# TianyiFranklinWang/MIRROR

Hardware: AMD Instinct MI355X
Metric: SSL samples/sec (slide+RNA pairs) (higher is better)
Workload: dtype bf16; 1 GPU; BASELINE c2: B=16/GPU x [4096 patch tokens x 1024-d] + [2048 genes], D=512, RNA depth 6 / 8 heads, train mode, local-batch InfoNCE; precision_policy=bf16, per_gpu_batch=16, global_batch=16, parallelism=dp1, grad_bucket_dtype=f32, step_launch=hip_graph

## Files before the change

### include/mirror_hip.h

```cpp
#ifndef MIRROR_HIP_H
#define MIRROR_HIP_H
#include <stdint.h>

#ifdef __cplusplus
extern "C" {
#endif

#define MH_OK 0
#define MH_EINVAL (-1)
#define MH_EUNSUP (-2)
#define MH_EHIP (-3)

#define MH_F32 0
#define MH_BF16 1

#define MH_ACT_NONE 0
#define MH_ACT_RELU 1
#define MH_ACT_GELU 2

typedef void* mh_stream;

const char* mh_last_error(void);
int mh_version(void);
int mh_exp_build(void);
// ... 122 lines not shown
                   int dt_v, int dt_o, mh_stream s);
int mh_resconv_wgrad(const void* v, int64_t ldv, int64_t v_bs, const void* dout, int64_t ldo, int64_t o_bs,
                     float* dw, int B, int n_p, int heads, int dh, int taps, int dt_v, int dt_o, mh_stream s);
int64_t mh_resconv_bwd_workspace_bytes(int B, int n_p, int heads, int dh, int taps);
int mh_resconv_bwd(const void* dout, int64_t ldo, int64_t o_bs, const void* v, int64_t ldv, int64_t v_bs, const float* w, void* dv,
                   int64_t lddv, int64_t dv_bs, float* dw, float* workspace, int64_t ws_floats, int B, int n_p, int heads, int dh,
                   int taps, int dt_v, int dt_o, mh_stream s);
int mh_pinv_absmax(const float* x, uint64_t* stats64, int BH, int m, mh_stream s);
int mh_pinv_z0(const float* x, const uint64_t* stats64, float* z0, int BH, int m, mh_stream s);
int mh_pinv_z0_bwd(const float* x, const float* z0, const float* dz0, const uint64_t* stats64, float* dx,
                   float* scratch1, int scratch_zeroed, int BH, int m, mh_stream s);
int mh_pinv_s2_bwd(const float* p, const float* dz0, const uint64_t* stats64, float* dx, float* scratch1, int scratch_zeroed, int BH,
                   int m, const float* mlm, int heads, mh_stream s);
int mh_pinv_chain_prep(const float* x, const uint64_t* stats64, float* z0, void* xp, void* z0p, int BH, int m, mh_stream s);
int mh_pinv_chain_pack(const float* dz, void* up, int BH, int m, mh_stream s);
int mh_pinv_chain_fwd(const void* XP, void* saved, void* zfT, int BH, int m, int iters, const float* z0f, const uint64_t* stats64,
                      int z0_rowmajor, mh_stream s);
int mh_nys_sim2(const void* lm, float* a2, void* xp, float* z0f, uint64_t* stats64, int B, int m, int D, int heads, float scale,
                int64_t lm_ld, const float* mlm, mh_stream s);
int mh_nys_dz_dav(const float* dw2, const float* av, const void* zfT, void* up, void* dav, float* delta3, int BH, int m, int dh,
                  mh_stream s);
int mh_pinv_chain_bwd(const void* XP, const void* saved, const void* dzf, void* work, float* dX, float* dz0, int BH, int m,
                      int iters, mh_stream s);
int64_t mh_pinv_chain_workspace_bytes(int BH, int m, int iters, int which);
int mh_nys_attn1_fwd(const void* qkv, const void* lm, const void* w2, void* out, float* lse1, const float* mrow, const float* mlm,
                     int B, int h, int n_p, int m, int dh, float scale, int accumulate, int64_t lm_ld, void* o1, mh_stream s);
int mh_nys_attn1_fwd_q8(const void* qkv, const void* lm, const void* w2, void* out, float* lse1, int B, int h, int n_p, int m, int dh,
                        float scale, int accumulate, void* q8, unsigned* ring, const float* tick, float margin, float* q8_scale, void* o1,
                        mh_stream s);
int64_t mh_nys_attn3_ws_floats(int B, int h, int n_p);
int64_t mh_nys_attn3_workspace_bytes(int B, int h, int n_p);
int mh_nys_attn3_fwd(const void* qkv, const void* lm, float* av, float* lse3, float* workspace, int64_t ws_floats,
                     const float* mrow, const float* mlm, int B, int h, int n_p, int m, int dh, float scale, int64_t lm_ld,
                     const float* rc_w, void* rc_out, mh_stream s);
int mh_nys_attn1_bwd(const void* qkv, const void* lm, const void* w2, const void* dout, const float* lse1, const void* o1, float* delta1,
                     void* dqkv, float* dw2, float* dlm, const float* mrow, const float* mlm, int B, int h, int n_p, int m, int dh,
                     float scale, int64_t lm_ld, mh_stream s);
int mh_nys_attn3_bwd(const void* qkv, const void* lm, const float* av, const void* dav, const float* lse3, float* delta3,
                     void* dqkv, float* dlm, const float* mrow, const float* mlm, int B, int h, int n_p, int m, int dh,
                     float scale, int64_t lm_ld, mh_stream s);
int mh_nys_cls_attn(const void* qkv, const void* lm, const void* z, const float* lse3, float* row, const float* mrow, const float* mlm,
                    int B, int h, int n_p, int m, int dh, int cls_row, float scale, int64_t lm_ld, int z_colmajor, int dt,
                    mh_stream s);
int mh_lm_merge(const float* a, const float* b, void* out, int64_t rows, int cols, int64_t out_ld, int zero_cols, mh_stream s);
int mh_eye_minus(const float* P, float* T, float d, int BH, int m, mh_stream s);

// ... 240 lines not shown
```

### mirror_amd/_lib.py

```python
from __future__ import annotations

import ctypes as C
import os

_HERE = os.path.dirname(os.path.abspath(__file__))
LIB_PATH = os.environ.get("MIRROR_HIP_LIB") or os.path.join(_HERE, "lib", "libmirror_hip.so")

MH_F32, MH_BF16 = 0, 1
ACT_NONE, ACT_RELU, ACT_GELU = 0, 1, 2


class GemmEpi(C.Structure):
    _fields_ = [
        ("kind", C.c_int32), ("resid", C.c_void_p),
        ("p", C.c_float), ("seed", C.c_uint64), ("offset", C.c_uint64), ("dev_base", C.c_void_p),
        ("mask", C.c_void_p), ("token", C.c_void_p), ("pos", C.c_void_p),
        ("rows_per_batch", C.c_int32), ("first", C.c_int32),
        ("tgt", C.c_void_p), ("tgt_bs", C.c_int64), ("sq", C.c_void_p),
    ]


class SkinnyWgradItem(C.Structure):
    _fields_ = [("dy", C.c_void_p), ("lddy", C.c_int64), ("x", C.c_void_p), ("ldx", C.c_int64), ("dw", C.c_void_p), ("lddw", C.c_int64),
                ("db", C.c_void_p), ("M", C.c_int32), ("N", C.c_int32), ("K", C.c_int32), ("dt_dy", C.c_int32), ("dt_x", C.c_int32)]
# ... 82 lines not shown
    "mh_layernorm_bwd": [P, P, P, P, P, P, P, P, I, I, I, L, L, I, I, I, I, P, L],
    "mh_layernorm_bwd_fan": [P, P, P, P, P, P, P, P, I, I, I, L, L, I, I, P, L, P, F, P],
    "mh_layernorm_bwd_drop": [P, P, P, P, P, P, P, P, I, I, I, L, L, I, I, P, L, P, F, P, P, F, U64, U64, P, P, I],
    "mh_layernorm_bwd_lm": [P, P, P, P, P, P, P, P, I, I, I, L, L, I, I, I, I, P, L, P, I, I, P, I, I, P, P, P],
    "mh_layernorm_fwd_lm": [P, P, P, P, P, P, P, P, I, I, I, L, I, I, F, P, P],
    "mh_softmax_fwd": [P, P, L, I, L, L, I, I],
    "mh_softmax_bwd": [P, P, P, L, I, L, L, L, I, I, I],
    "mh_landmark_fwd": [P, P, I, I, I, I, I],
    "mh_landmark_bwd": [P, P, I, I, I, I, I],
    "mh_resconv_fwd": [P, L, L, P, P, L, L, I, I, I, I, I, I, I, I, I],
    "mh_resconv_wgrad": [P, L, L, P, L, L, P, I, I, I, I, I, I, I],
    "mh_resconv_bwd": [P, L, L, P, L, L, P, P, L, L, P, P, L, I, I, I, I, I, I, I],
    "mh_pinv_absmax": [P, P, I, I],
    "mh_pinv_z0": [P, P, P, I, I],
    "mh_pinv_z0_bwd": [P, P, P, P, P, P, I, I, I],
    "mh_pinv_s2_bwd": [P, P, P, P, P, I, I, I, P, I],
    "mh_eye_minus": [P, P, F, I, I],
    "mh_pinv_chain_prep": [P, P, P, P, P, I, I],
    "mh_pinv_chain_pack": [P, P, I, I],
    "mh_pinv_chain_fwd": [P, P, P, I, I, I, P, P, I],
    "mh_nys_sim2": [P, P, P, P, P, I, I, I, I, F, L, P],
    "mh_nys_dz_dav": [P, P, P, P, P, P, I, I, I],
    "mh_pinv_chain_bwd": [P, P, P, P, P, P, I, I, I],
    "mh_nys_attn1_fwd": [P, P, P, P, P, P, P, I, I, I, I, I, F, I, L, P],
    "mh_nys_attn1_fwd_q8": [P, P, P, P, P, I, I, I, I, I, F, I, P, P, P, F, P, P],
    "mh_nys_attn3_fwd": [P, P, P, P, P, L, P, P, I, I, I, I, I, F, L, P, P],
    "mh_nys_attn1_bwd": [P, P, P, P, P, P, P, P, P, P, P, P, I, I, I, I, I, F, L],
    "mh_nys_attn3_bwd": [P, P, P, P, P, P, P, P, P, P, I, I, I, I, I, F, L],
    "mh_nys_cls_attn": [P, P, P, P, P, P, P, I, I, I, I, I, I, F, L, I, I],
    "mh_seq_finish": [P, P, I, I, I, I, I],
    "mh_seq_finish_bwd": [P, P, I, I, I, I, I],
    "mh_ppeg_merge": [P, P, P, P, P, P, P, P, I],
    "mh_ppeg_fwd": [P, P, P, P, I, I, I, I, I, I],
    "mh_ppeg_wgrad": [P, P, P, P, I, I, I, I, I],
    "mh_ppeg_grad_scatter": [P, P, P, P, P, P, P, P, I],
    "mh_rank_mask": [P, P, I, I, I],
    "mh_mask_apply_fwd": [P, P, P, P, P, I, I, I, I, I, I, I],
    "mh_mask_apply_bwd": [P, P, P, P, P, I, I, I, I, I, I, I, P],
    "mh_headattn_fwd": [P, P, P, I, I, I, I],
    "mh_headattn_bwd": [P, P, P, P, I, I, I, I],
    "mh_add": [P, P, P, L, I, I, I],
    "mh_lm_merge": [P, P, P, L, I, L, I],
    "mh_cast": [P, P, L, I, I],
    "mh_gelu_fwd": [P, P, L, I, I],
    "mh_gelu_bwd": [P, P, P, L, I, I, I],
    "mh_relu_bwd": [P, P, P, L, I, L, L, L, I, I, I],
# ... 161 lines not shown
```

### mirror_amd/csrc/nystrom_sim2.hip

```cpp
#include <cstdlib>
#include "gemm_kernel.h"

namespace {

#ifndef SIM2_EXP
#define SIM2_EXP 0
#endif
constexpr int SM = 256;
constexpr int SDH = 64;
constexpr long SMAT = (long)SM * SM;

template <int CTRL>
__device__ __forceinline__ float dpp_f(float v) {
    return __builtin_bit_cast(float, __builtin_amdgcn_update_dpp(0, __builtin_bit_cast(int, v), CTRL, 0xf, 0xf, true));
}
__device__ __forceinline__ float swz16_f(float v) {
    return __builtin_bit_cast(float, __builtin_amdgcn_ds_swizzle(__builtin_bit_cast(int, v), 0x401F));
}
__device__ __forceinline__ float half_max(float v) {
    v = fmaxf(v, dpp_f<0xB1>(v));
    v = fmaxf(v, dpp_f<0x4E>(v));
    v = fmaxf(v, dpp_f<0x141>(v));
    v = fmaxf(v, dpp_f<0x140>(v));
    return fmaxf(v, swz16_f(v));
// ... 153 lines not shown
#pragma unroll
            for (int e = 0; e < 16; e++) c[e] = __builtin_amdgcn_exp2f(c[e] * sl2 - mxi) * ivi;
#pragma unroll
            for (int t = 0; t < 2; t++) {
                float* dst = z0b + ((long)(cb * 16 + 2 * (2 * wave + rb) + t) * 64 + lane) * 8;
                *reinterpret_cast<f32x4*>(dst) = f32x4{c[8 * t], c[8 * t + 1], c[8 * t + 2], c[8 * t + 3]};
                *reinterpret_cast<f32x4*>(dst + 4) = f32x4{c[8 * t + 4], c[8 * t + 5], c[8 * t + 6], c[8 * t + 7]};
            }
        }
    }
    __syncthreads();
    if (tid < 2) atomicMax(stats + tid, s_best[tid]);
}

constexpr int DWP = 72;
constexpr int DTP = 264;
__device__ __forceinline__ bf16x8 cvt8(const float* p) {
    const f32x4 a = *reinterpret_cast<const f32x4*>(p), b = *reinterpret_cast<const f32x4*>(p + 4);
    bf16x8 o;
#pragma unroll
    for (int e = 0; e < 4; e++) { o[e] = (__bf16)a[e]; o[4 + e] = (__bf16)b[e]; }
    return o;
}
__global__ __launch_bounds__(256) void nys_dz_dav_kernel(const float* __restrict__ dw2, const float* __restrict__ av,
                                                         const bf16_t* __restrict__ zfT, bf16_t* __restrict__ up, bf16_t* __restrict__ dav,
                                                         float* __restrict__ delta3) {
    __shared__ __attribute__((aligned(16))) bf16_t s_dw[SM * DWP];
    __shared__ __attribute__((aligned(16))) bf16_t s_dt[SDH * DTP];
    const int tid = threadIdx.x, lane = tid & 63, r = lane & 31, hl = lane >> 5;
    const int wave = __builtin_amdgcn_readfirstlane(tid >> 6);
    const int bh = blockIdx.x;
    const int rb = blockIdx.y;
    const float* dwb = dw2 + (long)bh * SM * SDH;
    const float* avb = av + (long)bh * SM * SDH;
    bf16x8 af[4];
#pragma unroll
    for (int ks = 0; ks < 4; ks++) af[ks] = cvt8(avb + (long)(32 * (2 * wave + rb) + r) * SDH + 16 * ks + 8 * hl);
    bf16x8 zf[16];
#pragma unroll
    for (int ks = 0; ks < 16; ks++)
        zf[ks] = *reinterpret_cast<const bf16x8*>(zfT + (long)bh * SMAT + (long)(32 * (2 * wave + rb) + r) * SM + 16 * ks + 8 * hl);
#pragma unroll
    for (int n = 0; n < 16; n++) {
        const int e0 = 4 * (tid + 256 * n), i = e0 >> 6, d = e0 & 63;
        const f32x4 v = *reinterpret_cast<const f32x4*>(dwb + e0);
        unsigned short h[4];
#pragma unroll
        for (int e = 0; e < 4; e++) h[e] = f2bf(v[e]);
        *reinterpret_cast<u32x2*>(s_dw + i * DWP + d) = u32x2{(unsigned)h[0] | ((unsigned)h[1] << 16), (unsigned)h[2] | ((unsigned)h[3] << 16)};
#pragma unroll
        for (int e = 0; e < 4; e++) s_dt[(d + e) * DTP + i] = h[e];
    }
    __syncthreads();
    bf16_t* upb = up + (long)bh * SMAT;
#pragma unroll
        for (int cb = 0; cb < 8; cb++) {
            f32x16 c;
#pragma unroll
            for (int e = 0; e < 16; e++) c[e] = 0.f;
#pragma unroll
            for (int ks = 0; ks < 4; ks++) {
                const bf16x8 b = *reinterpret_cast<const bf16x8*>(s_dw + (32 * cb + r) * DWP + 16 * ks + 8 * hl);
                c = __builtin_amdgcn_mfma_f32_32x32x16_bf16(af[ks], b, c, 0, 0, 0);
            }
#pragma unroll
            for (int t = 0; t < 2; t++)
                *reinterpret_cast<u32x4*>(upb + ((cb * 16 + 2 * (2 * wave + rb) + t) * 512) + (lane << 3)) = pack8(c, t);
        }
    bf16_t* davb = dav + (long)bh * SM * SDH;
    {
        float dl[16];
#pragma unroll
        for (int reg = 0; reg < 16; reg++) dl[reg] = 0.f;
#pragma unroll
        for (int nb = 0; nb < 2; nb++) {
            f32x16 c;
#pragma unroll
            for (int e = 0; e < 16; e++) c[e] = 0.f;
#pragma unroll
            for (int ks = 0; ks < 16; ks++) {
                const bf16x8 b = *reinterpret_cast<const bf16x8*>(s_dt + (32 * nb + r) * DTP + 16 * ks + 8 * hl);
                c = __builtin_amdgcn_mfma_f32_32x32x16_bf16(zf[ks], b, c, 0, 0, 0);
            }
#pragma unroll
            for (int reg = 0; reg < 16; reg++) {
                const int row = 32 * (2 * wave + rb) + (reg & 3) + 8 * (reg >> 2) + 4 * hl;
                const unsigned short o = f2bf(c[reg]);
                davb[(long)row * SDH + 32 * nb + r] = o;
                if (delta3) dl[reg] += __uint_as_float((unsigned)o << 16) * avb[(long)row * SDH + 32 * nb + r];
            }
        }
        if (delta3) {
#pragma unroll
            for (int reg = 0; reg < 16; reg++) {
                const float d = half_sum(dl[reg]);
                if (r == 0) delta3[(long)bh * SM + 32 * (2 * wave + rb) + (reg & 3) + 8 * (reg >> 2) + 4 * hl] = d;
            }
        }
    }
}

}

extern "C" int mh_nys_sim2(const void* lm, float* a2, void* xp, float* z0f, uint64_t* stats64, int B, int m, int D, int heads, float scale,
                           int64_t lm_ld, const float* mlm, mh_stream s) {
    MH_REQUIRE(lm_ld == 0 || (lm_ld >= 2L * D && lm_ld % 8 == 0), "mh_nys_sim2: lm_ld must be 0 (contiguous [B, m, 2D]) or a multiple of 8 >= 2 D");
    MH_REQUIRE(m == SM && heads >= 1 && D == heads * SDH, "mh_nys_sim2: built for m = %d landmarks and dh = %d (m=%d, D=%d, heads=%d)", SM, SDH, m, D, heads);
    MH_REQUIRE(lm && a2 && xp && stats64 && (((uintptr_t)lm | (uintptr_t)a2 | (uintptr_t)xp | (uintptr_t)z0f) & 15) == 0,
               "mh_nys_sim2: null / unaligned buffer");
    MH_REQUIRE((long)B * heads * m < (1L << 31), "mh_nys_sim2: index overflow");
    if (B == 0) return MH_OK;
    if (mlm) {
        MH_REQUIRE(z0f == nullptr, "mh_nys_sim2: the masked form has no second pass (z0f must be NULL: the chain forms z_0 from attn2's rows)");
        hipLaunchKernelGGL(nys_sim2_kernel<true>, dim3(B * heads, 1), dim3(256), 0, (hipStream_t)s, (const bf16_t*)lm, lm_ld > 0 ? (long)lm_ld : 2L * D, D, heads, scale * 1.4426950408889634f,
                           a2, (bf16_t*)xp, z0f, (unsigned long long*)stats64, mlm);
        MH_LAUNCH_CHECK("mh_nys_sim2");
        return MH_OK;
    }
    hipLaunchKernelGGL(nys_sim2_kernel<false>, dim3(B * heads, 1), dim3(256), 0, (hipStream_t)s, (const bf16_t*)lm, lm_ld > 0 ? (long)lm_ld : 2L * D, D, heads, scale * 1.4426950408889634f,
                       a2, (bf16_t*)xp, z0f, (unsigned long long*)stats64, (const float*)nullptr);
    MH_LAUNCH_CHECK("mh_nys_sim2");
    return MH_OK;
}

extern "C" int mh_nys_dz_dav(const float* dw2, const float* av, const void* zfT, void* up, void* dav, float* delta3, int BH, int m, int dh,
                             mh_stream s) {
    MH_REQUIRE(m == SM && dh == SDH, "mh_nys_dz_dav: built for m = %d landmarks and dh = %d (m=%d, dh=%d)", SM, SDH, m, dh);
    MH_REQUIRE(dw2 && av && zfT && up && dav && (((uintptr_t)dw2 | (uintptr_t)av | (uintptr_t)zfT | (uintptr_t)up | (uintptr_t)dav) & 15) == 0,
               "mh_nys_dz_dav: null / unaligned buffer");
    if (BH == 0) return MH_OK;
    hipLaunchKernelGGL(nys_dz_dav_kernel, dim3(BH, 2), dim3(256), 0, (hipStream_t)s, dw2, av, (const bf16_t*)zfT, (bf16_t*)up, (bf16_t*)dav, delta3);
    MH_LAUNCH_CHECK("mh_nys_dz_dav");
    return MH_OK;
}
```

### mirror_amd/csrc/pinv_panel.hip

```cpp
#include "gemm_kernel.h"
#include <cstdlib>

#ifndef EXP
#define EXP 0
#endif

namespace {

constexpr int CM = 256;
constexpr int CT = 256;
constexpr int NJ = 2;
constexpr int NCH = CM * CM / 8 / CT;
constexpr long MAT = (long)CM * CM;
constexpr int IMG = CM * CM * 2;
typedef __attribute__((address_space(3))) s16x4 lds_s16x4;
typedef short s16x8 __attribute__((ext_vector_type(8)));
#define MFMA(a, b, c) __builtin_amdgcn_mfma_f32_32x32x16_bf16((a), (b), (c), 0, 0, 0)

__device__ __forceinline__ int swz(int k) { return ((k >> 1) & 7) | ((k & 1) << 3) | (((k >> 1) & 1) << 4); }

__device__ __forceinline__ bf16x8 tr_pair(const char* img, unsigned lo, unsigned hi) {
    s16x4 a = __builtin_amdgcn_ds_read_tr16_b64_v4i16((lds_s16x4*)(img + lo));
    s16x4 b = __builtin_amdgcn_ds_read_tr16_b64_v4i16((lds_s16x4*)(img + hi));
    s16x8 v = __builtin_shufflevector(a, b, 0, 1, 2, 3, 4, 5, 6, 7);
// ... 347 lines not shown
        finish<true>(acc, 1.f, 15.f, p, -7.f, p, wave, dreg);
        store_panel<true>(T2, p, wave, lane);
        panel_gemm<true>(acc, img, rlo, rhi, p);
        finish<false>(acc, -1.f, 13.f, p, 0.f, p, wave, dreg);
        store_panel<true>(T3, p, wave, lane);
        publish();
        image_from_global<16>(img, base, tid);
        __syncthreads();
        panel_gemm<true>(acc, img, rlo, rhi, p);
        finish<false>(acc, 0.25f, 0.f, p, 0.f, p, wave, dreg);
        if (k + 1 < iters) {
            store_panel(saved + ((long)(k + 1) * 4 * BH + bh) * MAT, p, wave, lane);
            publish();
            image_from_global<16>(img, Xb, tid);
        }
        __syncthreads();
    }
    image_from_panel(img, p, j, hl);
    __syncthreads();
    image_to_global(img, zfT + bh * MAT, tid);
}


__global__ __launch_bounds__(CT) void pinv_panel_bwd2_kernel(const bf16_t* __restrict__ XT, const bf16_t* __restrict__ saved,
                                                             const bf16_t* __restrict__ dzf, bf16_t* __restrict__ work,
                                                             float* __restrict__ dX, float* __restrict__ dz0, int BH, int iters) {
    __shared__ __attribute__((aligned(16))) char img[IMG];
    const int tid = threadIdx.x, lane = tid & 63, hl = lane >> 5;
    const int wave = __builtin_amdgcn_readfirstlane(tid >> 6);
    const int j = 64 * wave + (lane & 31);
    const int bh = blockIdx.x;
    const int dreg = (hl == ((lane >> 2) & 1)) ? ((((lane & 31) >> 3) << 2) | (lane & 3)) : -1;
    unsigned rlo[2][4], rhi[2][4];
    read_bases(rlo, rhi, lane);
    const bf16_t* Xb = XT + bh * MAT;
    f32x16 acc[8][NJ];
    bf16x8 p[16][NJ];
    const bf16_t* U = dzf + bh * MAT;
    image_from_global<16>(img, U, tid);
    load_panel(p, saved + ((long)(iters - 1) * 4 * BH + bh) * MAT, wave, lane);
    __syncthreads();
#pragma unroll 1
    for (int k = iters - 1; k >= 0; k--) {
        const bf16_t* sb = saved + ((long)k * 4 * BH + bh) * MAT;
        const bf16_t* P = sb + (long)BH * MAT;
        const bf16_t* T2 = sb + 2L * BH * MAT;
        const bf16_t* T3 = sb + 3L * BH * MAT;
        const bf16_t* Zn = saved + ((long)(k > 0 ? k - 1 : 0) * 4 * BH + bh) * MAT;
        bf16_t* W = work + ((long)k * BH + bh) * MAT;
        bf16_t* V3 = work + ((long)iters * BH + bh) * MAT;
        bf16_t* V2 = work + ((long)(iters + 1) * BH + bh) * MAT;
        bf16_t* Un = work + ((long)(iters + 2 + (k & 1)) * BH + bh) * MAT;
        panel_gemm<true, true>(acc, img, rlo, rhi, p, P, wave, lane);
        __syncthreads();
        finish_out<false>(acc, 0.25f, 0.f, p, 0.f, V3, img, wave, dreg, j, hl, lane);
        __syncthreads();
        panel_gemm<true, false>(acc, img, rlo, rhi, p);
        __syncthreads();
        finish_out<false>(acc, -1.f, 0.f, p, 0.f, V2, img, wave, dreg, j, hl, lane);
        __syncthreads();
        panel_gemm<true, true>(acc, img, rlo, rhi, p, V3, wave, lane);
        negate_panel(p);
        image_swap<true>(img, T2, tid);
        panel_gemm<false, true>(acc, img, rlo, rhi, p, V2, wave, lane);
        image_swap<true>(img, P, tid);
        panel_gemm<false, false>(acc, img, rlo, rhi, p);
        __syncthreads();
        finish_out<true, true, true>(acc, 4.f, 0.f, p, -28.f, W, img, wave, dreg, j, hl, lane, Xb);
        __syncthreads();
        panel_gemm<true, true>(acc, img, rlo, rhi, p, U, wave, lane);
        image_swap<true>(img, T3, tid);
        panel_gemm<false, false>(acc, img, rlo, rhi, p);
        load_panel(p, Zn, wave, lane);
        __syncthreads();
        finish_out<false>(acc, 0.25f, 0.f, p, 0.f, Un, img, wave, dreg, j, hl, lane);
        if (k == 0) store_f32(dz0 + bh * MAT, acc, 0.25f, j, hl);
        __syncthreads();
        U = Un;
    }
    zero_acc(acc);
    load_panel(p, work + ((long)bh) * MAT, wave, lane);
#pragma unroll 1
    for (int k = 0; k < iters; k++) {
        const bf16_t* Z = saved + ((long)k * 4 * BH + bh) * MAT;
        const bf16_t* Wn = work + ((long)(k + 1 < iters ? k + 1 : k) * BH + bh) * MAT;
        image_swap<true>(img, Z, tid);
        panel_gemm<false, true>(acc, img, rlo, rhi, p, Wn, wave, lane);
    }
    store_f32(dX + bh * MAT, acc, 0.25f, j, hl);
}


__device__ __forceinline__ void pn_item(int it, int& j, int& i0) {
    const int lane = it & 63, T = (it >> 6) & 15, jblk = it >> 10;
    j = 32 * jblk + (lane & 31);
    i0 = 16 * T + 4 * (lane >> 5);
}
__device__ __forceinline__ u32x4 pack_bf16x8(const float (&v)[8]) {
    u32x4 o;
#pragma unroll
    for (int w = 0; w < 4; w++) o[w] = pack_bf2(v[2 * w], v[2 * w + 1]);
    return o;
}

__global__ __launch_bounds__(256) void pinv_chain_prep_kernel(const float* __restrict__ x, const unsigned long long* __restrict__ st,
                                                              float* __restrict__ z0, bf16_t* __restrict__ xp,
                                                              bf16_t* __restrict__ z0p) {
    const float c = __uint_as_float((unsigned)(st[0] >> 32)), r = __uint_as_float((unsigned)(st[1] >> 32));
    const float inv = 1.f / (c * r);
    const int it = blockIdx.x * 256 + threadIdx.x;
    const long base = (long)blockIdx.y * MAT;
    int j, i0;
// ... 54 lines not shown
#endif
    MH_REQUIRE(!z0f || (stats64 && ((uintptr_t)z0f & 15) == 0), "mh_pinv_chain_fwd: z0f needs the maxima and 16-byte alignment");
    hipLaunchKernelGGL(pinv_panel_fwd_kernel, dim3(BH), dim3(CT), 0, (hipStream_t)s, (const bf16_t*)XT, (bf16_t*)saved,
                       (bf16_t*)zfT, BH, iters, z0f, (const unsigned long long*)stats64, z0_rowmajor);
    MH_LAUNCH_CHECK("mh_pinv_chain_fwd");
    return MH_OK;
}

extern "C" int mh_pinv_chain_bwd(const void* XT, const void* saved, const void* dzf, void* work, float* dX, float* dz0, int BH,
                                 int m, int iters, mh_stream s) {
    MH_REQUIRE(m == CM, "mh_pinv_chain_bwd: m=%d unsupported (built for m = %d; other sizes use mh_gemm)", m, CM);
    MH_REQUIRE(iters >= 1 && BH >= 0, "mh_pinv_chain_bwd: bad arguments");
    if (BH == 0) return MH_OK;
#ifdef MH_EXP
    if (getenv("MH_EXP_CHAIN_SKIP")) return MH_OK;
    if (const char* e = getenv("MH_EXP_CHAIN_BWD_ITERS")) iters = atoi(e);
#endif
    hipLaunchKernelGGL(pinv_panel_bwd2_kernel, dim3(BH), dim3(CT), 0, (hipStream_t)s, (const bf16_t*)XT, (const bf16_t*)saved,
                       (const bf16_t*)dzf, (bf16_t*)work, dX, dz0, BH, iters);
    MH_LAUNCH_CHECK("mh_pinv_chain_bwd");
    return MH_OK;
}

extern "C" int64_t mh_pinv_chain_workspace_bytes(int BH, int m, int iters, int which) {
    if (BH <= 0 || m != CM || iters < 1 || which < 0 || which > 1) return 0;
    return (which == 0 ? (int64_t)iters * 4 : (int64_t)iters + 4) * BH * MAT * 2;
}
```

### mirror_amd/functional.py

```python
from __future__ import annotations

from dataclasses import dataclass
from typing import List, Optional, Tuple

import os

import torch
from torch.autograd import Function

from . import kernels as K
from ._lib import ACT_NONE, ACT_RELU, MH_BF16, MH_F32

f32, bf16 = torch.float32, torch.bfloat16


@dataclass(frozen=True)
class Precision:
    name: str
    mma: int
    act: torch.dtype
    pinv_mma: int
    fp8_fwd: bool = False


# ... 1752 lines not shown
        ql, kl = _heads(lm, 0, 2, h), _heads(lm, 1, 2, h)
        dO = _heads(dout, 0, 1, h)
        de = dlm_out = None
        if ctx.lm_ext and A == bf16:
            de, dqkv, dlm_out = ext_rows_alloc(Bn, n_p, m, D3, 2 * D, qkv.device)
        else:
            dqkv = torch.empty_like(qkv)
        dq, dk, dv = (_heads(dqkv, i, 3, h) for i in range(3))
        rw = res_w.detach().contiguous()
        dres, dres_sunk = _gbuf(res_w, (rw.numel(),))
        if fused:
            lse1, lse3 = a1, a3
            dW2 = zeros((Bn, h, m, dh), qkv.device)
            dlm = zeros((Bn, m, 2 * D), qkv.device)
            delta1 = torch.empty_like(lse1)
            K.nys_attn1_bwd(qkv, lm, w2, dout, lse1, o1, delta1, dqkv, dW2, dlm, h, scale, kmask)
        else:
            dW2 = K.gemm(tr(a1), dO, mma=mma, out_dtype=f32)
            dlm = torch.empty((Bn, m, 2 * D), device=qkv.device, dtype=f32)
        dql, dkl = _heads(dlm, 0, 2, h), _heads(dlm, 1, 2, h)
        sd = f32 if pm == MH_F32 else bf16
        pio = pm if (pm == MH_BF16 or A == f32) else mma
        one2 = (chain and fused and A == bf16 and pio == MH_BF16 and dh == 64 and m == 256 and dW2.dtype == f32 and av.dtype == f32)
        dAV = dzb = None
        if one2:
            dzb, dAV = K.nys_dz_dav(dW2, av.contiguous(), zfT)
        else:
            dZ = K.gemm(dW2, tr(av), mma=pm, out_dtype=bf16 if (ctx.tile and _PINV_R32 and iters >= 1) else f32)
        side = dlm2 = None
        if chain:
            xb, chain_saved, z0 = flat
            work = K.pinv_chain_work_alloc(iters, Bn * h, m, qkv.device)
            dS2 = torch.empty_like(a2)
            dz0 = torch.empty_like(a2)
            if dzb is None:
                dzb = K.pinv_chain_pack(dZ)
            if fused and (kmask is None or _SIM2_MASKED):
                dlm2 = torch.empty_like(dlm)
            side = _side_stream(qkv.device)
            side.wait_stream(torch.cuda.current_stream())
            with torch.cuda.stream(side):
                K.pinv_chain_bwd(xb, chain_saved, dzb, work, dS2, dz0, iters)
                if (kmask is None or _SIM2_MASKED) and not ctx.z0_stored and a2.shape[-1] == 256:
                    K.pinv_s2_bwd(a2, dz0, st, dS2, _zeroed1(a2.device), mlm=mlm if kmask else None, heads=h)
                else:
                    K.pinv_z0_bwd(a2, z0 if ctx.z0_stored else None, dz0, st, dS2, _zeroed1(a2.device))
                    sm_bwd(a2, dS2, mlm if kmask else None, mlm if kmask else None)
                if dlm2 is not None:
                    K.gemm(tr(dS2), ql, out=_heads(dlm2, 1, 2, h), alpha=scale, mma=pio)
                    K.gemm(dS2, kl, out=_heads(dlm2, 0, 2, h), alpha=scale, mma=pio)
            K.shared_chip = True
        tile_side = ctx.tile and _TILE_SIDE and not chain
        if tile_side:
            dZ_ready = torch.cuda.current_stream().record_event()
            side = _side_stream(qkv.device)
            with torch.cuda.stream(side):
                side.wait_event(dZ_ready)
                dS2 = pinv_backward_tile(a2, saved, st, dZ, getattr(ctx, "a2b", None))
                sm_bwd(a2, dS2, mlm if kmask else None, mlm if kmask else None)
        if ctx.link is not None:
            ctx.link.run("wgrad")
        rc_bwd_one = fused and _RC_FUSED and A == bf16
        if not rc_bwd_one:
            K.resconv_wgrad(qkv[..., 2 * D:], dout, dres, h)
        if dAV is None:
            dAV = K.gemm(tr(zf), dW2, mma=pio, out_dtype=A)
        if fused:
            K.nys_attn3_bwd(qkv, lm, av, dAV, lse3, dqkv, dlm, h, scale, kmask)
            if rc_bwd_one:
                K.resconv_bwd(dout, qkv[..., 2 * D:], rw, dqkv[..., 2 * D:], dres, h)
            else:
                K.resconv(dout, rw, dqkv[..., 2 * D:], h, transpose=True, accumulate=True)
        else:
            if (kmask is None and A == bf16 and mma == MH_BF16 and a1.dtype == bf16 and a1.is_contiguous()
                    and K.gemm_softmax_ok(n_p, m, dh, dO.dtype, w2.dtype)):
                dS1 = K.gemm(dO, tr(w2), mma=mma, out_dtype=bf16, softmax_bwd_of=a1)
            else:
                dS1 = K.gemm(dO, tr(w2), mma=mma, out_dtype=A)
                sm_bwd(a1, dS1, mrow if kmask else None, mlm if kmask else None)
            dS3 = K.gemm(dAV, tr(v), mma=mma, out_dtype=A)
            K.gemm(tr(a3), dAV, out=dv, mma=mma)
            K.resconv(dout, rw, dqkv[..., 2 * D:], h, transpose=True, accumulate=True)
            sm_bwd(a3, dS3, mlm if kmask else None, mrow if kmask else None)
            K.gemm(dS1, kl, out=dq, alpha=scale, mma=mma)
            K.gemm(tr(dS3), ql, out=dk, alpha=scale, mma=mma)
            K.gemm(tr(dS1), q, out=dkl, alpha=scale, mma=mma)
            K.gemm(dS3, k, out=dql, alpha=scale, mma=mma)
        if tile_side:
            torch.cuda.current_stream().wait_stream(side)
        elif side is not None:
            torch.cuda.current_stream().wait_stream(side)
# ... 720 lines not shown
```

### mirror_amd/kernels.py

```python
from __future__ import annotations

import ctypes as C
import os
from typing import Optional


import torch

from . import _lib
from ._lib import ACT_GELU, ACT_NONE, ACT_RELU, MH_BF16, MH_F32, GemmDesc, MirrorHipError

_DT = {torch.float32: MH_F32, torch.bfloat16: MH_BF16}


def dt(t: torch.Tensor) -> int:
    try:
        return _DT[t.dtype]
    except KeyError:
        raise MirrorHipError(f"unsupported dtype {t.dtype} (f32 / bf16 only)") from None


_raw_stream = getattr(torch._C, "_cuda_getCurrentRawStream", None)


# ... 789 lines not shown
    _chk(x, stats, z0cm_out)
    _contig(x, "pinv_chain_prep input")
    m = x.shape[-1]
    BH = x.numel() // (m * m)
    if x.dtype != torch.float32 or z0cm_out.dtype != torch.bfloat16 or not z0cm_out.is_contiguous() or z0cm_out.numel() != x.numel():
        raise MirrorHipError("pinv_chain_prep: bad operands")
    z0 = torch.empty_like(x)
    xt = torch.empty(x.shape, device=x.device, dtype=torch.bfloat16)
    _lib.call("mh_pinv_chain_prep", _p(x), _p(stats), _p(z0), _p(xt), _p(z0cm_out), BH, m, stream=_stream())
    return z0, xt


def pinv_chain_pack(dz: torch.Tensor) -> torch.Tensor:
    _chk(dz)
    _contig(dz, "pinv_chain_pack input")
    m = dz.shape[-1]
    if dz.dtype != torch.float32:
        raise MirrorHipError("pinv_chain_pack: f32 input expected")
    up = torch.empty(dz.shape, device=dz.device, dtype=torch.bfloat16)
    _lib.call("mh_pinv_chain_pack", _p(dz), _p(up), dz.numel() // (m * m), m, stream=_stream())
    return up


def nys_dz_dav(dw2: torch.Tensor, av: torch.Tensor, zfT: torch.Tensor, want_delta3: bool = False, out=None):
    _chk(dw2, av, zfT)
    m, dh = dw2.shape[-2], dw2.shape[-1]
    BH = dw2.numel() // (m * dh)
    if not (dw2.dtype == av.dtype == torch.float32 and zfT.dtype == torch.bfloat16 and dw2.is_contiguous() and av.is_contiguous()
            and zfT.is_contiguous() and av.shape == dw2.shape and zfT.numel() == BH * m * m):
        raise MirrorHipError("nys_dz_dav: contiguous f32 [.., m, dh] gradients / products and the bf16 column-major chain output")
    if out is None:
        up = torch.empty(zfT.shape, device=dw2.device, dtype=torch.bfloat16)
        dav = torch.empty(dw2.shape, device=dw2.device, dtype=torch.bfloat16)
    else:
        up, dav = out
        _chk(up, dav)
        if not (up.dtype == dav.dtype == torch.bfloat16 and up.is_contiguous() and dav.is_contiguous() and up.numel() == zfT.numel()
                and dav.shape == dw2.shape):
            raise MirrorHipError("nys_dz_dav: out must be contiguous bf16 buffers shaped like zfT and dw2")
    delta3 = torch.empty(dw2.shape[:-1], device=dw2.device, dtype=torch.float32) if want_delta3 else None
    _lib.call("mh_nys_dz_dav", _p(dw2), _p(av), _p(zfT), _p(up), _p(dav), _p(delta3), BH, m, dh, stream=_stream())
    return (up, dav, delta3) if want_delta3 else (up, dav)


_NYS_SIM2 = True


def nys_sim2_ok(lm: torch.Tensor, heads: int) -> bool:
    return (_NYS_SIM2 and lm.dim() == 3 and lm.dtype == torch.bfloat16 and _lm_ld(lm) > 0 and lm.shape[1] == PINV_CHAIN_M
            and lm.shape[2] == 2 * heads * 64)


def nys_sim2_alloc(lm: torch.Tensor, heads: int):
    Bn, m, _ = lm.shape
# ... 32 lines not shown
        raise MirrorHipError("pinv_chain_fwd: bad z0f / stats")
    fn = lambda: _lib.call("mh_pinv_chain_fwd", _p(XT), _p(saved), _p(zfT), BH, m, iters, _p(z0f), _p(stats), int(z0_rowmajor), stream=_stream())
    if gemm_profiler is None:
        fn()
    else:
        gemm_profiler.launch_named("pinv_panel_fwd_kernel", iters * 4 * 2.0 * m ** 3 * BH, fn)


def pinv_chain_bwd(XT, saved, dzf, work, dX, dz0, iters: int) -> None:
    _chk(XT, saved, dzf, work, dX, dz0)
    m = XT.shape[-1]
    BH = XT.numel() // (m * m)
    bf = torch.bfloat16
    if not (all(t.dtype == bf and t.is_contiguous() for t in (XT, saved, dzf, work))
            and all(t.dtype == torch.float32 and t.is_contiguous() and t.numel() == BH * m * m for t in (dX, dz0))
            and saved.numel() == iters * 4 * BH * m * m and work.numel() >= (iters + 4) * BH * m * m and dzf.numel() == BH * m * m):
        raise MirrorHipError("pinv_chain_bwd: bad operands")
    fn = lambda: _lib.call("mh_pinv_chain_bwd", _p(XT), _p(saved), _p(dzf), _p(work), _p(dX), _p(dz0), BH, m, iters,
                           stream=_stream())
    if gemm_profiler is None:
        fn()
    else:
        gemm_profiler.launch_named("pinv_panel_bwd2_kernel", iters * 8 * 2.0 * m ** 3 * BH, fn)


NYS_FUSED_M, NYS_FUSED_DH = 256, 64


def nys_fused_ok(qkv: torch.Tensor, heads: int, m: int) -> bool:
    D = qkv.shape[-1] // 3
    return qkv.dtype == torch.bfloat16 and D == heads * NYS_FUSED_DH and m == NYS_FUSED_M and qkv.shape[1] % m == 0


def _nys_check(name: str, B: int, h: int, n_p: int, **tensors) -> None:
    D = h * NYS_FUSED_DH
    want = {"qkv": ((B, n_p, 3 * D), torch.bfloat16), "dqkv": ((B, n_p, 3 * D), torch.bfloat16),
            "lm": ((B, NYS_FUSED_M, 2 * D), torch.bfloat16), "dlm": ((B, NYS_FUSED_M, 2 * D), torch.float32),
            "w2": ((B, h, NYS_FUSED_M, NYS_FUSED_DH), torch.bfloat16), "dw2": ((B, h, NYS_FUSED_M, NYS_FUSED_DH), torch.float32),
            "av": ((B, h, NYS_FUSED_M, NYS_FUSED_DH), torch.float32), "dav": ((B, h, NYS_FUSED_M, NYS_FUSED_DH), torch.bfloat16),
            "out": ((B, n_p, D), torch.bfloat16), "dout": ((B, n_p, D), torch.bfloat16), "o1": ((B, n_p, D), torch.bfloat16),
            "lse1": ((B, h, n_p), torch.float32), "delta1": ((B, h, n_p), torch.float32),
            "lse3": ((B, h, NYS_FUSED_M), torch.float32)}
    for k, t in tensors.items():
        shape, dtype = want[k]
        if k == "lm" and tuple(t.shape) == shape and t.dtype == dtype and _lm_ld(t) > 0:
            continue
# ... 1173 lines not shown
```

Baseline: 2201 samples/s.

## Fuse dZ outer product into pinv chain backward kernel prologue

Computes dZ = dW2·AVᵀ inside the pinv chain backward kernel's prologue, on the side stream, instead of writing a packed dZ buffer from a separate kernel and reading it back. The main stream then runs a reduced kernel that produces only dAV and delta3. This removes one m×m bf16 round trip per head and moves the dZ work onto the side stream so it can overlap. The cost is more prologue work and register pressure in the chain kernel, plus a new code path used only when there is no mask and z0 is not stored.

```diff
diff --git a/include/mirror_hip.h b/include/mirror_hip.h
--- a/include/mirror_hip.h
+++ b/include/mirror_hip.h
@@ -168,6 +168,8 @@
                   mh_stream s);
 int mh_pinv_chain_bwd(const void* XP, const void* saved, const void* dzf, void* work, float* dX, float* dz0, int BH, int m,
                       int iters, mh_stream s);
+int mh_pinv_chain_bwd_fused(const void* XP, const void* saved, const float* dw2, const float* av, void* work, float* dX, float* dz0,
+                            int BH, int m, int dh, int iters, mh_stream s);
 int64_t mh_pinv_chain_workspace_bytes(int BH, int m, int iters, int which);
 int mh_nys_attn1_fwd(const void* qkv, const void* lm, const void* w2, void* out, float* lse1, const float* mrow, const float* mlm,
                      int B, int h, int n_p, int m, int dh, float scale, int accumulate, int64_t lm_ld, void* o1, mh_stream s);
diff --git a/mirror_amd/_lib.py b/mirror_amd/_lib.py
--- a/mirror_amd/_lib.py
+++ b/mirror_amd/_lib.py
@@ -128,6 +128,7 @@
     "mh_nys_sim2": [P, P, P, P, P, I, I, I, I, F, L, P],
     "mh_nys_dz_dav": [P, P, P, P, P, P, I, I, I],
     "mh_pinv_chain_bwd": [P, P, P, P, P, P, I, I, I],
+    "mh_pinv_chain_bwd_fused": [P, P, P, P, P, P, P, I, I, I, I],
     "mh_nys_attn1_fwd": [P, P, P, P, P, P, P, I, I, I, I, I, F, I, L, P],
     "mh_nys_attn1_fwd_q8": [P, P, P, P, P, I, I, I, I, I, F, I, P, P, P, F, P, P],
     "mh_nys_attn3_fwd": [P, P, P, P, P, L, P, P, I, I, I, I, I, F, L, P, P],
diff --git a/mirror_amd/csrc/nystrom_sim2.hip b/mirror_amd/csrc/nystrom_sim2.hip
--- a/mirror_amd/csrc/nystrom_sim2.hip
+++ b/mirror_amd/csrc/nystrom_sim2.hip
@@ -199,11 +199,10 @@
     for (int e = 0; e < 4; e++) { o[e] = (__bf16)a[e]; o[4 + e] = (__bf16)b[e]; }
     return o;
 }
-__global__ __launch_bounds__(256) void nys_dz_dav_kernel(const float* __restrict__ dw2, const float* __restrict__ av,
-                                                         const bf16_t* __restrict__ zfT, bf16_t* __restrict__ up, bf16_t* __restrict__ dav,
-                                                         float* __restrict__ delta3) {
-    __shared__ __attribute__((aligned(16))) bf16_t s_dw[SM * DWP];
-    __shared__ __attribute__((aligned(16))) bf16_t s_dt[SDH * DTP];
+template <bool DZ>
+__device__ __forceinline__ void nys_dz_dav_body(bf16_t* s_dw, bf16_t* s_dt, const float* __restrict__ dw2, const float* __restrict__ av,
+                                                const bf16_t* __restrict__ zfT, bf16_t* __restrict__ up, bf16_t* __restrict__ dav,
+                                                float* __restrict__ delta3) {
     const int tid = threadIdx.x, lane = tid & 63, r = lane & 31, hl = lane >> 5;
     const int wave = __builtin_amdgcn_readfirstlane(tid >> 6);
     const int bh = blockIdx.x;
@@ -211,8 +210,10 @@
     const float* dwb = dw2 + (long)bh * SM * SDH;
     const float* avb = av + (long)bh * SM * SDH;
     bf16x8 af[4];
-#pragma unroll
-    for (int ks = 0; ks < 4; ks++) af[ks] = cvt8(avb + (long)(32 * (2 * wave + rb) + r) * SDH + 16 * ks + 8 * hl);
+    if constexpr (DZ) {
+#pragma unroll
+        for (int ks = 0; ks < 4; ks++) af[ks] = cvt8(avb + (long)(32 * (2 * wave + rb) + r) * SDH + 16 * ks + 8 * hl);
+    }
     bf16x8 zf[16];
 #pragma unroll
     for (int ks = 0; ks < 16; ks++)
@@ -224,11 +225,13 @@
         unsigned short h[4];
 #pragma unroll
         for (int e = 0; e < 4; e++) h[e] = f2bf(v[e]);
-        *reinterpret_cast<u32x2*>(s_dw + i * DWP + d) = u32x2{(unsigned)h[0] | ((unsigned)h[1] << 16), (unsigned)h[2] | ((unsigned)h[3] << 16)};
+        if constexpr (DZ)
+            *reinterpret_cast<u32x2*>(s_dw + i * DWP + d) = u32x2{(unsigned)h[0] | ((unsigned)h[1] << 16), (unsigned)h[2] | ((unsigned)h[3] << 16)};
 #pragma unroll
         for (int e = 0; e < 4; e++) s_dt[(d + e) * DTP + i] = h[e];
     }
     __syncthreads();
+    if constexpr (DZ) {
     bf16_t* upb = up + (long)bh * SMAT;
 #pragma unroll
         for (int cb = 0; cb < 8; cb++) {
@@ -244,6 +247,7 @@
             for (int t = 0; t < 2; t++)
                 *reinterpret_cast<u32x4*>(upb + ((cb * 16 + 2 * (2 * wave + rb) + t) * 512) + (lane << 3)) = pack8(c, t);
         }
+    }
     bf16_t* davb = dav + (long)bh * SM * SDH;
     {
         float dl[16];
@@ -275,6 +279,18 @@
             }
         }
     }
+}
+__global__ __launch_bounds__(256) void nys_dz_dav_kernel(const float* __restrict__ dw2, const float* __restrict__ av,
+                                                         const bf16_t* __restrict__ zfT, bf16_t* __restrict__ up, bf16_t* __restrict__ dav,
+                                                         float* __restrict__ delta3) {
+    __shared__ __attribute__((aligned(16))) bf16_t s_dw[SM * DWP];
+    __shared__ __attribute__((aligned(16))) bf16_t s_dt[SDH * DTP];
+    nys_dz_dav_body<true>(s_dw, s_dt, dw2, av, zfT, up, dav, delta3);
+}
+__global__ __launch_bounds__(256) void nys_dav_kernel(const float* __restrict__ dw2, const float* __restrict__ av,
+                                                      const bf16_t* __restrict__ zfT, bf16_t* __restrict__ dav, float* __restrict__ delta3) {
+    __shared__ __attribute__((aligned(16))) bf16_t s_dt[SDH * DTP];
+    nys_dz_dav_body<false>(nullptr, s_dt, dw2, av, zfT, nullptr, dav, delta3);
 }
 
 }
@@ -303,9 +319,14 @@
 extern "C" int mh_nys_dz_dav(const float* dw2, const float* av, const void* zfT, void* up, void* dav, float* delta3, int BH, int m, int dh,
                              mh_stream s) {
     MH_REQUIRE(m == SM && dh == SDH, "mh_nys_dz_dav: built for m = %d landmarks and dh = %d (m=%d, dh=%d)", SM, SDH, m, dh);
-    MH_REQUIRE(dw2 && av && zfT && up && dav && (((uintptr_t)dw2 | (uintptr_t)av | (uintptr_t)zfT | (uintptr_t)up | (uintptr_t)dav) & 15) == 0,
+    MH_REQUIRE(dw2 && av && zfT && dav && (((uintptr_t)dw2 | (uintptr_t)av | (uintptr_t)zfT | (uintptr_t)up | (uintptr_t)dav) & 15) == 0,
                "mh_nys_dz_dav: null / unaligned buffer");
     if (BH == 0) return MH_OK;
+    if (!up) {
+        hipLaunchKernelGGL(nys_dav_kernel, dim3(BH, 2), dim3(256), 0, (hipStream_t)s, dw2, av, (const bf16_t*)zfT, (bf16_t*)dav, delta3);
+        MH_LAUNCH_CHECK("mh_nys_dz_dav");
+        return MH_OK;
+    }
     hipLaunchKernelGGL(nys_dz_dav_kernel, dim3(BH, 2), dim3(256), 0, (hipStream_t)s, dw2, av, (const bf16_t*)zfT, (bf16_t*)up, (bf16_t*)dav, delta3);
     MH_LAUNCH_CHECK("mh_nys_dz_dav");
     return MH_OK;
diff --git a/mirror_amd/csrc/pinv_panel.hip b/mirror_amd/csrc/pinv_panel.hip
--- a/mirror_amd/csrc/pinv_panel.hip
+++ b/mirror_amd/csrc/pinv_panel.hip
@@ -393,10 +393,32 @@
 }
 
 
-__global__ __launch_bounds__(CT) void pinv_panel_bwd2_kernel(const bf16_t* __restrict__ XT, const bf16_t* __restrict__ saved,
-                                                             const bf16_t* __restrict__ dzf, bf16_t* __restrict__ work,
-                                                             float* __restrict__ dX, float* __restrict__ dz0, int BH, int iters) {
-    __shared__ __attribute__((aligned(16))) char img[IMG];
+template <int T>
+__device__ __forceinline__ void k64_step(f32x16 (&acc)[8][NJ], bf16x8 (&cur)[8], bf16x8 (&nxt)[8], const char* img,
+                                         const unsigned (&blo)[2][4], const unsigned (&bhi)[2][4], const bf16x8 (&pB)[16][NJ]) {
+    if constexpr (T + 1 < 4) load_frags<T + 1>(nxt, img, blo, bhi);
+    __builtin_amdgcn_sched_barrier(0);
+#pragma unroll
+    for (int blk = 0; blk < 8; blk++)
+#pragma unroll
+        for (int jb = 0; jb < NJ; jb++) {
+            if constexpr (T == 0) {
+                f32x16 z;
+#pragma unroll
+                for (int r = 0; r < 16; r++) z[r] = 0.f;
+                acc[blk][jb] = MFMA(cur[blk], pB[T][jb], z);
+            } else {
+                acc[blk][jb] = MFMA(cur[blk], pB[T][jb], acc[blk][jb]);
+            }
+        }
+    __builtin_amdgcn_sched_barrier(0);
+}
+
+template <bool PRO>
+__device__ __forceinline__ void pinv_panel_bwd2_body(char* img, const bf16_t* __restrict__ XT, const bf16_t* __restrict__ saved,
+                                                     const bf16_t* __restrict__ dzf, bf16_t* __restrict__ work,
+                                                     float* __restrict__ dX, float* __restrict__ dz0, int BH, int iters,
+                                                     const float* __restrict__ dw2, const float* __restrict__ av) {
     const int tid = threadIdx.x, lane = tid & 63, hl = lane >> 5;
     const int wave = __builtin_amdgcn_readfirstlane(tid >> 6);
     const int j = 64 * wave + (lane & 31);
@@ -407,10 +429,60 @@
     const bf16_t* Xb = XT + bh * MAT;
     f32x16 acc[8][NJ];
     bf16x8 p[16][NJ];
-    const bf16_t* U = dzf + bh * MAT;
-    image_from_global<16>(img, U, tid);
-    load_panel(p, saved + ((long)(iters - 1) * 4 * BH + bh) * MAT, wave, lane);
-    __syncthreads();
+    const bf16_t* U;
+    if constexpr (PRO) {
+        bf16_t* U0 = work + ((long)(iters + 2 + (iters & 1)) * BH + bh) * MAT;
+        U = U0;
+        {
+            const float* avb = av + (long)bh * CM * 64;
+            const int i4 = tid & 63, dq = tid >> 6;
+            f32x4 r[4][4];
+#pragma unroll
+            for (int e = 0; e < 4; e++)
+#pragma unroll
+                for (int q = 0; q < 4; q++) r[e][q] = *reinterpret_cast<const f32x4*>(avb + (4 * i4 + e) * 64 + 16 * dq + 4 * q);
+#pragma unroll
+            for (int q = 0; q < 4; q++)
+#pragma unroll
+                for (int c = 0; c < 4; c++) {
+                    const int row = 16 * dq + 4 * (q == 1 ? 2 : q == 2 ? 1 : q) + c;
+                    *reinterpret_cast<u32x2*>(img + row * 512 + ((i4 ^ swz(row)) << 3)) =
+                        u32x2{pack_bf2(r[0][q][c], r[1][q][c]), pack_bf2(r[2][q][c], r[3][q][c])};
+                }
+        }
+        {
+            const float* dwb = dw2 + (long)bh * CM * 64;
+#pragma unroll
+            for (int jb = 0; jb < NJ; jb++)
+#pragma unroll
+                for (int T = 0; T < 4; T++) {
+                    const float* src = dwb + (j + 32 * jb) * 64 + 16 * T + 8 * hl;
+                    const f32x4 a = *reinterpret_cast<const f32x4*>(src), b = *reinterpret_cast<const f32x4*>(src + 4);
+                    bf16x8 o;
+#pragma unroll
+                    for (int e = 0; e < 4; e++) { o[e] = (__bf16)a[e]; o[4 + e] = (__bf16)b[e]; }
+                    p[T][jb] = o;
+                }
+        }
+        __syncthreads();
+        {
+            bf16x8 f0[8], f1[8];
+            load_frags<0>(f0, img, rlo, rhi);
+            k64_step<0>(acc, f0, f1, img, rlo, rhi, p);
+            k64_step<1>(acc, f1, f0, img, rlo, rhi, p);
+            k64_step<2>(acc, f0, f1, img, rlo, rhi, p);
+            k64_step<3>(acc, f1, f0, img, rlo, rhi, p);
+        }
+        load_panel(p, saved + ((long)(iters - 1) * 4 * BH + bh) * MAT, wave, lane);
+        __syncthreads();
+        finish_out<false>(acc, 1.f, 0.f, p, 0.f, U0, img, wave, dreg, j, hl, lane);
+        __syncthreads();
+    } else {
+        U = dzf + bh * MAT;
+        image_from_global<16>(img, U, tid);
+        load_panel(p, saved + ((long)(iters - 1) * 4 * BH + bh) * MAT, wave, lane);
+        __syncthreads();
+    }
 #pragma unroll 1
     for (int k = iters - 1; k >= 0; k--) {
         const bf16_t* sb = saved + ((long)k * 4 * BH + bh) * MAT;
@@ -449,7 +521,18 @@
         __syncthreads();
         U = Un;
     }
-    zero_acc(acc);
+    if constexpr (PRO) {
+        float z = 0.f;
+        asm volatile("" : "+v"(z));
+#pragma unroll
+        for (int blk = 0; blk < 8; blk++)
+#pragma unroll
+            for (int jb = 0; jb < NJ; jb++)
+#pragma unroll
+                for (int r = 0; r < 16; r++) acc[blk][jb][r] = z;
+    } else {
+        zero_acc(acc);
+    }
     load_panel(p, work + ((long)bh) * MAT, wave, lane);
 #pragma unroll 1
     for (int k = 0; k < iters; k++) {
@@ -459,6 +542,20 @@
         panel_gemm<false, true>(acc, img, rlo, rhi, p, Wn, wave, lane);
     }
     store_f32(dX + bh * MAT, acc, 0.25f, j, hl);
+}
+
+__global__ __launch_bounds__(CT) void pinv_panel_bwd2_kernel(const bf16_t* __restrict__ XT, const bf16_t* __restrict__ saved,
+                                                             const bf16_t* __restrict__ dzf, bf16_t* __restrict__ work,
+                                                             float* __restrict__ dX, float* __restrict__ dz0, int BH, int iters) {
+    __shared__ __attribute__((aligned(16))) char img[IMG];
+    pinv_panel_bwd2_body<false>(img, XT, saved, dzf, work, dX, dz0, BH, iters, nullptr, nullptr);
+}
+__global__ __launch_bounds__(CT) void pinv_panel_bwd2_dz_kernel(const bf16_t* __restrict__ XT, const bf16_t* __restrict__ saved,
+                                                                const float* __restrict__ dw2, const float* __restrict__ av,
+                                                                bf16_t* __restrict__ work, float* __restrict__ dX, float* __restrict__ dz0,
+                                                                int BH, int iters) {
+    __shared__ __attribute__((aligned(16))) char img[IMG];
+    pinv_panel_bwd2_body<true>(img, XT, saved, nullptr, work, dX, dz0, BH, iters, dw2, av);
 }
 
 
@@ -559,6 +656,24 @@
     return MH_OK;
 }
 
+extern "C" int mh_pinv_chain_bwd_fused(const void* XT, const void* saved, const float* dw2, const float* av, void* work, float* dX,
+                                       float* dz0, int BH, int m, int dh, int iters, mh_stream s) {
+    MH_REQUIRE(m == CM && dh == 64, "mh_pinv_chain_bwd_fused: built for m = %d, dh = 64 (m=%d, dh=%d): compose mh_nys_dz_dav + mh_pinv_chain_bwd", CM, m, dh);
+    MH_REQUIRE(iters >= 1 && BH >= 0, "mh_pinv_chain_bwd_fused: bad arguments");
+    MH_REQUIRE(XT && saved && dw2 && av && work && dX && dz0 &&
+               (((uintptr_t)XT | (uintptr_t)saved | (uintptr_t)dw2 | (uintptr_t)av | (uintptr_t)work | (uintptr_t)dX | (uintptr_t)dz0) & 15) == 0,
+               "mh_pinv_chain_bwd_fused: null / unaligned buffer");
+    if (BH == 0) return MH_OK;
+#ifdef MH_EXP
+    if (getenv("MH_EXP_CHAIN_SKIP")) return MH_OK;
+    if (const char* e = getenv("MH_EXP_CHAIN_BWD_ITERS")) iters = atoi(e);
+#endif
+    hipLaunchKernelGGL(pinv_panel_bwd2_dz_kernel, dim3(BH), dim3(CT), 0, (hipStream_t)s, (const bf16_t*)XT, (const bf16_t*)saved, dw2, av,
+                       (bf16_t*)work, dX, dz0, BH, iters);
+    MH_LAUNCH_CHECK("mh_pinv_chain_bwd_fused");
+    return MH_OK;
+}
+
 extern "C" int64_t mh_pinv_chain_workspace_bytes(int BH, int m, int iters, int which) {
     if (BH <= 0 || m != CM || iters < 1 || which < 0 || which > 1) return 0;
     return (which == 0 ? (int64_t)iters * 4 : (int64_t)iters + 4) * BH * MAT * 2;
diff --git a/mirror_amd/functional.py b/mirror_amd/functional.py
--- a/mirror_amd/functional.py
+++ b/mirror_amd/functional.py
@@ -1798,8 +1798,11 @@
         sd = f32 if pm == MH_F32 else bf16
         pio = pm if (pm == MH_BF16 or A == f32) else mma
         one2 = (chain and fused and A == bf16 and pio == MH_BF16 and dh == 64 and m == 256 and dW2.dtype == f32 and av.dtype == f32)
-        dAV = dzb = None
-        if one2:
+        pro = one2 and kmask is None and not ctx.z0_stored
+        dAV = dzb = delta3 = None
+        if pro:
+            av = av.contiguous()
+        elif one2:
             dzb, dAV = K.nys_dz_dav(dW2, av.contiguous(), zfT)
         else:
             dZ = K.gemm(dW2, tr(av), mma=pm, out_dtype=bf16 if (ctx.tile and _PINV_R32 and iters >= 1) else f32)
@@ -1809,14 +1812,17 @@
             work = K.pinv_chain_work_alloc(iters, Bn * h, m, qkv.device)
             dS2 = torch.empty_like(a2)
             dz0 = torch.empty_like(a2)
-            if dzb is None:
+            if dzb is None and not pro:
                 dzb = K.pinv_chain_pack(dZ)
             if fused and (kmask is None or _SIM2_MASKED):
                 dlm2 = torch.empty_like(dlm)
             side = _side_stream(qkv.device)
             side.wait_stream(torch.cuda.current_stream())
             with torch.cuda.stream(side):
-                K.pinv_chain_bwd(xb, chain_saved, dzb, work, dS2, dz0, iters)
+                if pro:
+                    K.pinv_chain_bwd_fused(xb, chain_saved, dW2, av, work, dS2, dz0, iters)
+                else:
+                    K.pinv_chain_bwd(xb, chain_saved, dzb, work, dS2, dz0, iters)
                 if (kmask is None or _SIM2_MASKED) and not ctx.z0_stored and a2.shape[-1] == 256:
                     K.pinv_s2_bwd(a2, dz0, st, dS2, _zeroed1(a2.device), mlm=mlm if kmask else None, heads=h)
                 else:
@@ -1826,6 +1832,8 @@
                     K.gemm(tr(dS2), ql, out=_heads(dlm2, 1, 2, h), alpha=scale, mma=pio)
                     K.gemm(dS2, kl, out=_heads(dlm2, 0, 2, h), alpha=scale, mma=pio)
             K.shared_chip = True
+            if pro:
+                _, dAV, delta3 = K.nys_dz_dav(dW2, av, zfT, want_delta3=True, dav_only=True)
         tile_side = ctx.tile and _TILE_SIDE and not chain
         if tile_side:
             dZ_ready = torch.cuda.current_stream().record_event()
@@ -1842,7 +1850,7 @@
         if dAV is None:
             dAV = K.gemm(tr(zf), dW2, mma=pio, out_dtype=A)
         if fused:
-            K.nys_attn3_bwd(qkv, lm, av, dAV, lse3, dqkv, dlm, h, scale, kmask)
+            K.nys_attn3_bwd(qkv, lm, av, dAV, lse3, dqkv, dlm, h, scale, kmask, delta3=delta3)
             if rc_bwd_one:
                 K.resconv_bwd(dout, qkv[..., 2 * D:], rw, dqkv[..., 2 * D:], dres, h)
             else:
diff --git a/mirror_amd/kernels.py b/mirror_amd/kernels.py
--- a/mirror_amd/kernels.py
+++ b/mirror_amd/kernels.py
@@ -835,14 +835,19 @@
     return up
 
 
-def nys_dz_dav(dw2: torch.Tensor, av: torch.Tensor, zfT: torch.Tensor, want_delta3: bool = False, out=None):
+def nys_dz_dav(dw2: torch.Tensor, av: torch.Tensor, zfT: torch.Tensor, want_delta3: bool = False, out=None, dav_only: bool = False):
     _chk(dw2, av, zfT)
     m, dh = dw2.shape[-2], dw2.shape[-1]
     BH = dw2.numel() // (m * dh)
     if not (dw2.dtype == av.dtype == torch.float32 and zfT.dtype == torch.bfloat16 and dw2.is_contiguous() and av.is_contiguous()
             and zfT.is_contiguous() and av.shape == dw2.shape and zfT.numel() == BH * m * m):
         raise MirrorHipError("nys_dz_dav: contiguous f32 [.., m, dh] gradients / products and the bf16 column-major chain output")
-    if out is None:
+    if dav_only:
+        if out is not None:
+            raise MirrorHipError("nys_dz_dav: dav_only allocates its result")
+        up = None
+        dav = torch.empty(dw2.shape, device=dw2.device, dtype=torch.bfloat16)
+    elif out is None:
         up = torch.empty(zfT.shape, device=dw2.device, dtype=torch.bfloat16)
         dav = torch.empty(dw2.shape, device=dw2.device, dtype=torch.bfloat16)
     else:
@@ -921,6 +926,24 @@
         fn()
     else:
         gemm_profiler.launch_named("pinv_panel_bwd2_kernel", iters * 8 * 2.0 * m ** 3 * BH, fn)
+
+
+def pinv_chain_bwd_fused(XT, saved, dw2, av, work, dX, dz0, iters: int) -> None:
+    _chk(XT, saved, dw2, av, work, dX, dz0)
+    m = XT.shape[-1]
+    BH = XT.numel() // (m * m)
+    bf = torch.bfloat16
+    if not (all(t.dtype == bf and t.is_contiguous() for t in (XT, saved, work))
+            and all(t.dtype == torch.float32 and t.is_contiguous() and t.numel() == BH * m * m for t in (dX, dz0))
+            and all(t.dtype == torch.float32 and t.is_contiguous() and t.numel() == BH * m * 64 for t in (dw2, av))
+            and saved.numel() == iters * 4 * BH * m * m and work.numel() >= (iters + 4) * BH * m * m):
+        raise MirrorHipError("pinv_chain_bwd_fused: bad operands")
+    fn = lambda: _lib.call("mh_pinv_chain_bwd_fused", _p(XT), _p(saved), _p(dw2), _p(av), _p(work), _p(dX), _p(dz0), BH, m, 64, iters,
+                           stream=_stream())
+    if gemm_profiler is None:
+        fn()
+    else:
+        gemm_profiler.launch_named("pinv_panel_bwd2_dz_kernel", (iters * 8 * 2.0 * m ** 3 + 2.0 * m * m * 64) * BH, fn)
 
 
 NYS_FUSED_M, NYS_FUSED_DH = 256, 64
```

Result: no change. 2193 samples/s (-0.3%).
